# mikemey/cellcomm

Hardware: NVIDIA B200
Metric: BiGAN train cells/sec (higher is better)
Workload: dtype bf16

## Files before the change

### cellcomm_b200/_lib.py

```python
import ctypes as C
import os

from . import build as _build

_LIB = None

c_i32, c_i64, c_u32, c_u64, c_f32 = C.c_int32, C.c_int64, C.c_uint32, C.c_uint64, C.c_float
vp = C.c_void_p


class GemmDesc(C.Structure):
    _fields_ = [
        ("M", c_i32), ("N", c_i32),
        ("a_mn_major", c_i32), ("b_mn_major", c_i32),
        ("nseg", c_i32),
        ("a", vp * 4), ("lda", c_i64 * 4),
        ("b", vp * 4), ("ldb", c_i64 * 4),
        ("k", c_i32 * 4),
        ("alpha", c_f32),
        ("bias", vp), ("act", c_i32),
        ("dact_y", vp), ("ld_dact", c_i64), ("dact", c_i32),
        ("out16", vp), ("ld16", c_i64), ("beta16", c_i32),
        ("out32", vp), ("ld32", c_i64), ("beta32", c_i32),
        ("workspace", vp), ("workspace_elems", c_i64),
        ("force_splits", c_i32), ("force_bn", c_i32),
        ("rms_p32", vp), ("rms_ms", vp), ("rms_mom", vp), ("rms_p16", vp), ("rms_ld", c_i64),
        ("rms_lr", c_f32), ("rms_rho", c_f32), ("rms_momentum", c_f32), ("rms_eps", c_f32),
        ("route_world", c_i32), ("route_shard", c_i64), ("route_off0", c_i64),
        ("route_base", vp * 16),
        ("out16_lo", vp), ("ld16_lo", c_i64),
        ("rms_blocked", c_i32), ("rms_row0", c_i32), ("rms_p16_lo", vp),
    ]


class PeerRmspropDesc(C.Structure):
    _fields_ = [
        ("world", c_i32), ("rank", c_i32),
        ("grad", vp * 16), ("p16", vp * 16),
        ("p32", vp), ("ms", vp), ("mom", vp),
        ("start", c_i64), ("count", c_i64),
        ("broadcast", c_i32),
        ("lr", c_f32), ("rho", c_f32), ("momentum", c_f32), ("eps", c_f32),
        ("ready", vp), ("epoch", c_u32),
        ("epoch_ctr", vp),
        ("p16_multicast", vp),
        ("p16lo", vp * 16), ("p16lo_multicast", vp),
        ("lo_begin", c_i64 * 2), ("lo_end", c_i64 * 2),
    ]


ENC_MAX_OPS = ENC_MAX_SLOTS = 32
ENC_DENSE, ENC_SPLIT, ENC_COPY, ENC_BN_INFER, ENC_SOFTMAX = range(5)


class EncOp(C.Structure):
    _fields_ = [
        ("kind", c_i32), ("n_in", c_i32),
        ("in_", c_i32 * 4), ("w_row", c_i32 * 4),
        ("out", c_i32), ("out2", c_i32),
        ("width", c_i32), ("act", c_i32),
        ("w16", vp), ("ldw", c_i64),
        ("bias", vp),
        ("gamma", vp), ("beta", vp), ("mean", vp), ("var", vp),
        ("eps", c_f32),
# ... 13 lines not shown


SIGNATURES = {
    "cc_last_error": (C.c_char_p, []),
    "cc_version": (C.c_int, []),
    "cc_launch_count": (C.c_longlong, []),
    "cc_arch": (C.c_char_p, []),
    "cc_reload_env": (None, []),
    "cc_mtx_load_csr": (C.c_int, [C.c_char_p, C.POINTER(vp)]),
    "cc_coo_to_csr": (C.c_int, [vp, vp, vp, c_i64, C.POINTER(vp)]),
    "cc_csr_destroy": (None, [vp]),
    "cc_csr_rows": (c_i64, [vp]),
    "cc_csr_cols": (c_i64, [vp]),
    "cc_csr_nnz": (c_i64, [vp]),
    "cc_csr_rowptr": (vp, [vp]),
    "cc_csr_colidx": (vp, [vp]),
    "cc_csr_values": (vp, [vp]),
    "cc_csr_values64": (vp, [vp]),
    "cc_csr_row_ids": (vp, [vp]),
    "cc_csr_col_ids": (vp, [vp]),
    "cc_mtx_load_coo": (C.c_int, [C.c_char_p, C.POINTER(vp)]),
    "cc_coo_destroy": (None, [vp]),
    "cc_coo_nnz": (c_i64, [vp]),
    "cc_coo_gene": (vp, [vp]),
    "cc_coo_barcode": (vp, [vp]),
    "cc_coo_value": (vp, [vp]),
    "cc_coo_build_csr": (C.c_int, [vp, C.POINTER(vp)]),
    "cc_mtx_write": (C.c_int, [C.c_char_p, c_i64, c_i64, c_i64, vp, vp, vp, vp, vp]),
    "cc_encode_scratch_bytes": (c_i64, [C.POINTER(EncodePlan)]),
    "cc_encode_stream": (C.c_int, [vp, vp, vp, c_i64, c_i64, C.POINTER(EncodePlan), vp, c_i64, vp]),
    "cc_gather_rows": (C.c_int, [vp, vp, vp, vp, c_i64, c_i64, c_i64, vp, c_i64, vp, c_i64, vp]),
    "cc_gemm": (C.c_int, [C.POINTER(GemmDesc), vp]),
    "cc_gemm_workspace_elems": (c_i64, [c_i32, c_i32]),
    "cc_dense_fwd": (C.c_int, [c_i32, c_i32, c_i32, C.POINTER(vp), C.POINTER(c_i64),
                               C.POINTER(c_i32), C.POINTER(vp), C.POINTER(c_i64), vp, c_i32,
                               vp, c_i64, vp, c_i64, vp, c_i64, vp]),
    "cc_dense_dgrad": (C.c_int, [c_i32, c_i32, c_i32, C.POINTER(vp), C.POINTER(c_i64),
                                 C.POINTER(c_i32), C.POINTER(vp), C.POINTER(c_i64), vp, c_i64,
                                 c_i32, c_f32, vp, c_i64, c_i32, vp, c_i64, vp]),
    "cc_dense_wgrad": (C.c_int, [c_i32, c_i32, c_i32, vp, c_i64, vp, c_i64, vp, c_i64, c_i32, vp]),
    "cc_reduce_ws_floats": (c_i64, [c_i64, c_i64]),
    "cc_colsum": (C.c_int, [vp, c_i64, c_i64, c_i64, vp, c_i32, c_i32, vp]),
    "cc_colsum_ws": (C.c_int, [vp, c_i64, c_i64, c_i64, vp, c_i32, c_i32, vp, c_i64, vp]),
    "cc_bias_grad": (C.c_int, [vp, c_i64, vp, c_i64, c_i64, c_i64, c_i32, vp, c_i32, vp, c_i64, vp,
                               c_i64, c_i32, vp]),
    "cc_bias_grad_ws": (C.c_int, [vp, c_i64, vp, c_i64, c_i64, c_i64, c_i32, vp, c_i32, vp, c_i64,
                                  vp, c_i64, c_i32, vp, c_i64, vp]),
    "cc_split_bf16": (C.c_int, [vp, c_i64, vp, c_i64, vp, c_i64, c_i64, c_i64, c_i32, vp]),
    "cc_dropout": (C.c_int, [vp, c_i64, vp, c_i64, c_i64, c_i64, c_f32, vp, c_i64, c_u64, vp,
                             c_u32, c_i32, vp]),
    "cc_dropout_mask": (C.c_int, [vp, c_i64, c_i64, c_i64, c_f32, c_u64, vp, c_u32, vp]),
    "cc_uniform": (C.c_int, [vp, vp, c_i64, c_i64, c_i64, c_u64, vp, c_u32, vp]),
    "cc_counter_add": (C.c_int, [vp, c_u64, vp]),
    "cc_act_bwd": (C.c_int, [vp, c_i64, vp, c_i64, vp, c_i64, c_i64, c_i64, c_i32, c_i32, vp]),
    "cc_copy2d": (C.c_int, [vp, c_i64, vp, c_i64, c_i64, c_i64, c_i32, c_f32, c_i32, vp]),
    "cc_bn_stats": (C.c_int, [vp, c_i64, c_i64, c_i64, vp, c_i32, vp]),
    "cc_bn_stats_ws": (C.c_int, [vp, c_i64, c_i64, c_i64, vp, c_i32, vp, c_i64, vp]),
    "cc_bn_train_apply": (C.c_int, [vp, c_i64, vp, c_i64, c_i64, c_i64, vp, c_i64, vp, vp, c_f32,
                                    c_f32, vp, vp, vp, vp, c_i32, vp]),
    "cc_bn_infer": (C.c_int, [vp, c_i64, vp, c_i64, c_i64, c_i64, vp, vp, vp, vp, c_f32, c_i32,
                              vp]),
    "cc_bn_bwd_stats": (C.c_int, [vp, c_i64, vp, c_i64, c_i64, c_i64, vp, vp, vp, c_i32, vp]),
    "cc_bn_bwd_stats_ws": (C.c_int, [vp, c_i64, vp, c_i64, c_i64, c_i64, vp, vp, vp, c_i32, vp,
                                     c_i64, vp]),
    "cc_bn_bwd_apply": (C.c_int, [vp, c_i64, vp, c_i64, vp, c_i64, c_i64, c_i64, vp, vp, vp, vp,
                                  c_i64, vp, vp, c_i32, vp]),
# ... 62 lines not shown
```

### cellcomm_b200/csrc/gemm_sm100.cu

```cuda
#include <cuda.h>

#include <mutex>
#include <unordered_map>

#include "common.cuh"

namespace cc {

constexpr int BM = 128;
constexpr int BK = 64;
constexpr int UMMA_K = 16;
constexpr int MAX_SEG = CC_GEMM_MAX_SEG;

struct EpiParams {
  int M, N;
  float alpha;
  const float* bias;
  int act;
  const bf16* dact_y;
  long long ld_dact;
  int dact;
  bf16* out16;
  long long ld16;
  int beta16;
  bf16* out16_lo;
  long long ld16_lo;
  float* out32;
  long long ld32;
  int beta32;
  float* rms_p32;
  float* rms_ms;
  float* rms_mom;
  bf16* rms_p16;
  long long rms_ld;
  float rms_lr, rms_rho, rms_momentum, rms_eps;
  int rms_cs;
  int rms_blocked;
  int rms_row0;
  bf16* rms_p16lo;
  int rms_keep_operands;
  int route_world;
  unsigned int route_shard;
  long long route_off0;
  float* route_base[CC_PEER_MAX];
};

struct GemmParams {
  EpiParams epi;
  int nseg;
  int kblocks[MAX_SEG];
  int total_kblocks;
  int kb_per_split;
  int psplits;
  float* partial;
  long long partial_ld;
  long long partial_stride;
  unsigned long long adesc_hi, bdesc_hi;
  unsigned int a_kstep, b_kstep;
  unsigned int idesc;
  int bn_eff;
  int b_boxes;
  int b_half_rows;
  int cluster;
  int pair;
  unsigned int stage_tx;
};

struct TmaMaps {
  CUtensorMap a[MAX_SEG];
  CUtensorMap b[MAX_SEG];
};

__device__ __forceinline__ uint32_t smem_u32(const void* p) {
  return (uint32_t)__cvta_generic_to_shared(p);
}
__device__ __forceinline__ void mbar_init(uint32_t bar, uint32_t count) {
  asm volatile("mbarrier.init.shared::cta.b64 [%0], %1;" ::"r"(bar), "r"(count));
}
// ... 977 lines not shown
}

}
#include "wgrad_rmsprop_kernel.cuh"
namespace cc {

__global__ void splitk_finalize_kernel(const EpiParams e, const float* __restrict__ partial,
                                       long long partial_ld, long long partial_stride, int splits) {
  const int groups = (e.N + 3) / 4;
  const long long idx = (long long)blockIdx.x * blockDim.x + threadIdx.x;
  if (idx >= (long long)e.M * groups) return;
  const int r = (int)(idx / groups);
  const int c0 = (int)(idx % groups) * 4;
  const float* src = partial + (long long)r * partial_ld + c0;
  float4 a = make_float4(0.f, 0.f, 0.f, 0.f);
  for (int s0 = 0; s0 < splits; s0 += 8) {
    float4 q[8];
#pragma unroll
    for (int u = 0; u < 8; ++u)
      q[u] = (s0 + u < splits)
                 ? __ldcs(reinterpret_cast<const float4*>(src + (long long)(s0 + u) * partial_stride))
                 : make_float4(0.f, 0.f, 0.f, 0.f);
#pragma unroll
    for (int u = 0; u < 8; ++u) {
      if (s0 + u < splits) {
        a.x += q[u].x;
        a.y += q[u].y;
        a.z += q[u].z;
        a.w += q[u].w;
      }
    }
  }
  float v[4] = {a.x, a.y, a.z, a.w};
  const int ncols = min(4, e.N - c0);
#pragma unroll
  for (int j = 0; j < 4; ++j) {
    float x = v[j] * e.alpha;
    if (e.bias != nullptr && j < ncols) x += __ldg(e.bias + c0 + j);
    if (e.act == CC_ACT_SIGMOID) x = sigmoidf_(x);
    else if (e.act == CC_ACT_RELU) x = fmaxf(x, 0.f);
    v[j] = x;
  }
  if (e.dact != 0) {
    const bf16* yrow = e.dact_y + (long long)r * e.ld_dact + c0;
#pragma unroll
    for (int j = 0; j < 4; ++j) {
      if (j < ncols) {
        const float y = bf2f(yrow[j]);
        v[j] *= (e.dact == CC_ACT_SIGMOID) ? y * (1.f - y) : (y > 0.f ? 1.f : 0.f);
      }
    }
  }
  if (e.out32 != nullptr) {
    float* o = e.out32 + (long long)r * e.ld32 + c0;
    if (ncols == 4 && (((uintptr_t)o) & 15) == 0 && !e.beta32) {
      *reinterpret_cast<float4*>(o) = make_float4(v[0], v[1], v[2], v[3]);
    } else {
#pragma unroll
      for (int j = 0; j < 4; ++j)
        if (j < ncols) o[j] = e.beta32 ? o[j] + v[j] : v[j];
    }
  }
  if (e.out16 != nullptr) {
    bf16* o = e.out16 + (long long)r * e.ld16 + c0;
    if (ncols == 4 && (((uintptr_t)o) & 7) == 0 && !e.beta16) {
      __nv_bfloat162 p0 = __floats2bfloat162_rn(v[0], v[1]);
      __nv_bfloat162 p1 = __floats2bfloat162_rn(v[2], v[3]);
      uint2 u;
      u.x = *reinterpret_cast<uint32_t*>(&p0);
      u.y = *reinterpret_cast<uint32_t*>(&p1);
      *reinterpret_cast<uint2*>(o) = u;
    } else {
#pragma unroll
      for (int j = 0; j < 4; ++j)
        if (j < ncols) o[j] = f2bf(e.beta16 ? bf2f(o[j]) + v[j] : v[j]);
    }
    if (e.out16_lo != nullptr) {
      bf16* l = e.out16_lo + (long long)r * e.ld16_lo + c0;
#pragma unroll
      for (int j = 0; j < 4; ++j)
        if (j < ncols) l[j] = f2bf(v[j] - bf2f(f2bf(v[j])));
    }
  }
}

typedef CUresult (*PFN_encodeTiled)(CUtensorMap*, CUtensorMapDataType, cuuint32_t, void*,
                                    const cuuint64_t*, const cuuint64_t*, const cuuint32_t*,
                                    const cuuint32_t*, CUtensorMapInterleave, CUtensorMapSwizzle,
                                    CUtensorMapL2promotion, CUtensorMapFloatOOBfill);

static PFN_encodeTiled get_encode_fn() {
  static PFN_encodeTiled fn = nullptr;
  static std::once_flag once;
  std::call_once(once, [] {
    void* ptr = nullptr;
    cudaDriverEntryPointQueryResult qres;
    if (cudaGetDriverEntryPoint("cuTensorMapEncodeTiled", &ptr, cudaEnableDefault, &qres) ==
            cudaSuccess &&
        qres == cudaDriverEntryPointSuccess)
      fn = (PFN_encodeTiled)ptr;
  });
  return fn;
}

struct MapKey {
  const void* ptr;
  uint64_t inner, outer, ld;
  uint32_t box_inner, box_outer;
  uint32_t kind;
  bool operator==(const MapKey& o) const {
    return ptr == o.ptr && inner == o.inner && outer == o.outer && ld == o.ld &&
           box_inner == o.box_inner && box_outer == o.box_outer && kind == o.kind;
  }
};
struct MapKeyHash {
  size_t operator()(const MapKey& k) const {
// ... 330 lines not shown
  if (d->rms_blocked) {
    CC_REQUIRE(d->rms_p32 != nullptr && d->a_mn_major && d->b_mn_major && d->N > 128 &&
                   d->alpha == 1.f && d->bias == nullptr && d->act == 0 && d->dact_y == nullptr &&
                   d->out16 == nullptr && d->beta32 == 0 && d->route_world == 0 &&
                   d->force_splits <= 1 && (d->force_bn == 0 || d->force_bn == 256),
               "cc_gemm: rms_blocked is for plain weight-gradient GEMMs (X^T dZ, N > 128)");
    CC_REQUIRE(d->rms_row0 >= 0 && (d->rms_ld & 31) == 0 &&
                   ((((uintptr_t)d->rms_p32) | ((uintptr_t)d->rms_ms) | ((uintptr_t)d->rms_mom) |
                     ((uintptr_t)d->rms_p16) | ((uintptr_t)d->rms_p16_lo) | ((uintptr_t)d->out32)) & 15) == 0 &&
                   (d->out32 == nullptr || (d->ld32 & 3) == 0),
               "cc_gemm: rms_blocked needs 16-byte aligned blocks, rms_ld %% 32 == 0 (rms_ld=%lld)",
               (long long)d->rms_ld);
  }
  CC_REQUIRE(d->rms_p16_lo == nullptr || d->rms_blocked,
             "cc_gemm: rms_p16_lo is written by the blocked fused-optimiser epilogue only");
  if (d->route_world > 0) {
    CC_REQUIRE(d->out32 != nullptr && d->beta32 == 0 && d->workspace == nullptr &&
                   d->rms_p32 == nullptr,
               "cc_gemm: a routed output needs a plain fp32 output without split-K");
    CC_REQUIRE(d->route_shard > 0 && (d->route_shard & 7) == 0 && d->route_shard < (1ll << 32) &&
                   d->route_off0 >= 0 && (d->route_off0 & 3) == 0,
               "cc_gemm: route_shard=%lld route_off0=%lld", (long long)d->route_shard,
               (long long)d->route_off0);
    for (int q = 0; q < d->route_world; ++q)
      CC_REQUIRE(d->route_base[q] != nullptr, "cc_gemm: route_base[%d] is null", q);
  }
  if (g_num_sms == 0) {
    int dev = 0;
    CC_CHECK_CUDA(cudaGetDevice(&dev));
    CC_CHECK_CUDA(cudaDeviceGetAttribute(&g_num_sms, cudaDevAttrMultiProcessorCount, dev));
    const int cap = ENV.sms;
    if (cap >= 2 && cap < g_num_sms) g_num_sms = cap / 2 * 2;
  }
  const bool a_mn = d->a_mn_major != 0, b_mn = d->b_mn_major != 0;

  int bn = d->force_bn ? d->force_bn : ENV.bn;
  if (bn == 0) bn = (d->N > 128) ? 256 : 128;
  CC_REQUIRE(bn == 128 || bn == 256, "cc_gemm: BN=%d unsupported", bn);

  GemmParams p{};
  TmaMaps maps;
  memset(&maps, 0, sizeof(maps));
  p.nseg = d->nseg;
  int total = 0;
  for (int s = 0; s < d->nseg; ++s) {
    CC_REQUIRE(d->k[s] > 0, "cc_gemm: segment %d has k=%d", s, d->k[s]);
    p.kblocks[s] = (d->k[s] + BK - 1) / BK;
    total += p.kblocks[s];
  }
  p.total_kblocks = total;

  const int mt = (d->M + BM - 1) / BM;
  int nt = (d->N + bn - 1) / bn;
  int splits = 1;
  const long long Mpad = (long long)mt * BM, Npad = (long long)nt * bn;
  if (d->workspace != nullptr && d->rms_p32 == nullptr) {
    int want = d->force_splits ? d->force_splits : ENV.splits;
    if (want == 0) {
      const int tiles = mt * nt;
      if (2 * tiles <= g_num_sms && total >= 8) {
        want = (2 * g_num_sms) / tiles;
        if (want < 1) want = 1;
        if (want > total / 4) want = total / 4;
      } else {
        want = 1;
      }
// ... 50 lines not shown
  if (p.pair) {
    p.b_boxes = bn_eff / 128;
    p.stage_tx = (unsigned)(BM * BK * 2 + (bn_eff / 2) * BK * 2);
  }

  for (int s = 0; s < d->nseg; ++s) {
    int rc;
    if (a_mn)
      rc = make_map(&maps.a[s], d->a[s], (uint64_t)d->M, (uint64_t)d->k[s], (uint64_t)d->lda[s], 64, BK);
    else
      rc = make_map(&maps.a[s], d->a[s], (uint64_t)d->k[s], (uint64_t)d->M, (uint64_t)d->lda[s], BK, BM);
    if (rc) return rc;
    if (b_mn)
      rc = make_map(&maps.b[s], d->b[s], (uint64_t)d->N, (uint64_t)d->k[s], (uint64_t)d->ldb[s], 64, BK);
    else
      rc = make_map(&maps.b[s], d->b[s], (uint64_t)d->k[s], (uint64_t)d->N, (uint64_t)d->ldb[s], BK,
                    (uint32_t)(persistent ? (p.cluster == 2 ? bn_eff / 2 : bn_eff) : bn));
    if (rc) return rc;
  }

  const uint32_t mn_lbo = (uint32_t)ENV.mn_lbo;
  const uint32_t mn_sbo = (uint32_t)ENV.mn_sbo;
  const uint32_t mn_kstep = (uint32_t)ENV.mn_kstep;
  const uint32_t k_lbo = (uint32_t)ENV.k_lbo;
  const uint32_t k_sbo = (uint32_t)ENV.k_sbo;
  p.adesc_hi = a_mn ? desc_hi(mn_lbo, mn_sbo) : desc_hi(k_lbo, k_sbo);
  p.bdesc_hi = b_mn ? desc_hi(mn_lbo, mn_sbo) : desc_hi(k_lbo, k_sbo);
  p.a_kstep = a_mn ? mn_kstep : UMMA_K * 2;
  p.b_kstep = b_mn ? mn_kstep : UMMA_K * 2;
  p.idesc = (1u << 4) | (1u << 7) | (1u << 10) | ((a_mn ? 1u : 0u) << 15) |
            ((b_mn ? 1u : 0u) << 16) | ((uint32_t)((persistent ? bn_eff : bn) >> 3) << 17) |
            ((uint32_t)(((persistent && p.pair) ? 2 * BM : BM) >> 4) << 24);

  EpiParams& e = p.epi;
  e.M = d->M;
  e.N = d->N;
  e.alpha = d->alpha;
  e.bias = d->bias;
  e.act = d->act;
  e.dact_y = (const bf16*)d->dact_y;
  e.ld_dact = d->ld_dact;
  e.dact = d->dact_y ? d->dact : 0;
  e.out16 = (bf16*)d->out16;
  e.ld16 = d->ld16;
  e.beta16 = d->beta16;
  e.out16_lo = (bf16*)d->out16_lo;
  e.ld16_lo = d->ld16_lo;
  e.out32 = d->out32;
  e.ld32 = d->ld32;
  e.beta32 = d->beta32;
  e.rms_p32 = d->rms_p32;
  e.rms_ms = d->rms_ms;
  e.rms_mom = d->rms_mom;
  e.rms_p16 = (bf16*)d->rms_p16;
  e.rms_ld = d->rms_ld;
  e.rms_lr = d->rms_lr;
  e.rms_rho = d->rms_rho;
  e.rms_momentum = d->rms_momentum;
  e.rms_eps = d->rms_eps;
  e.rms_cs = (ENV.rms_cs ? 1 : 0) | (ENV.rms_l2_256 ? 8 : 0);
  e.rms_blocked = d->rms_blocked;
  e.rms_row0 = d->rms_row0;
  e.rms_p16lo = d->rms_blocked ? (bf16*)d->rms_p16_lo : nullptr;
  e.rms_keep_operands = ENV.rms_keep;
  e.route_world = d->route_world;
  e.route_shard = (unsigned)d->route_shard;
  e.route_off0 = d->route_off0;
  for (int q = 0; q < CC_PEER_MAX; ++q)
    e.route_base[q] = q < d->route_world ? d->route_base[q] : nullptr;

  if (persistent) {
    if (bn == 256 && d->rms_p32 != nullptr && a_mn && b_mn && d->alpha == 1.f &&
        d->bias == nullptr && d->act == 0 && e.dact == 0 && ENV.rms_warps == 8) {
      int nfast = ENV.rms_nfast;
      if (nfast < 0) nfast = ((long long)total * BK * d->N * 2 <= (48ll << 20)) ? 1 : 0;
      if (d->rms_blocked) {
        if (p.cluster == 2)
          return nfast ? launch_persistent_one<256, 4, true, true, false, 8, true, 2, false, true>(
                             maps, p, mt, nt, g_num_sms, st)
                       : launch_persistent_one<256, 4, true, true, false, 8, false, 2, false, true>(
                             maps, p, mt, nt, g_num_sms, st);
        return nfast ? launch_persistent_one<256, 4, true, true, false, 8, true, 1, false, true>(
                           maps, p, mt, nt, g_num_sms, st)
// ... 106 lines not shown
```

### cellcomm_b200/ops.py

```python
import ctypes as C

import torch

from . import _lib
from ._lib import GemmDesc, check

COMPUTE_DTYPE = torch.bfloat16
ACT_NONE, ACT_SIGMOID, ACT_RELU = 0, 1, 2
ACT_IDS = {None: 0, "none": 0, "linear": 0, "sigmoid": 1, "relu": 2}


def _stream():
    return torch.cuda.current_stream().cuda_stream


def _req(t, dtype, name):
    if t is None:
        return
    if not t.is_cuda:
        raise RuntimeError(f"cellcomm_b200.ops: {name} must be a CUDA tensor (no CPU fallback)")
    if t.dtype != dtype:
        raise TypeError(f"cellcomm_b200.ops: {name} must be {dtype}, got {t.dtype}")
    if t.dim() == 2 and t.shape[1] > 1 and t.stride(1) != 1:
        raise ValueError(f"cellcomm_b200.ops: {name} must be row-major (stride(1)==1)")
# ... 7 lines not shown
    if t is None:
        return 0
    if t.dim() == 1:
        return t.shape[0]
    return t.stride(0) if t.shape[0] > 1 else max(t.stride(0), t.shape[1])


def pad_ld(cols, mult=64):
    return max(mult, (cols + mult - 1) // mult * mult)


def alloc2d(rows, cols, dtype=torch.bfloat16, device="cuda", zero=True):
    ld = pad_ld(cols)
    buf = (torch.zeros if zero else torch.empty)((max(rows, 1), ld), dtype=dtype, device=device)
    return buf[:rows, :cols]


_WS = {}


def workspace(device):
    key = str(device)
    ws = _WS.get(key)
    if ws is None:
        ws = torch.empty(296 * 128 * 256 * 2, dtype=torch.float32, device=device)
        _WS[key] = ws
    return ws


def launch_count():
    return int(_lib.load().cc_launch_count())


def reload_env():
    _lib.load().cc_reload_env()


def gemm(M, N, a_list, b_list, k_list, a_mn, b_mn, *, bias=None, act=0, dact_y=None, dact=0,
         alpha=1.0, out16=None, beta16=0, out32=None, beta32=0, splits=0, bn=0, use_ws=True,
         rms=None, route=None, out16_lo=None, rms_row0=None, rms_lo=None):
    lib = _lib.load()
    d = GemmDesc()
    d.M, d.N = int(M), int(N)
    d.a_mn_major, d.b_mn_major = int(a_mn), int(b_mn)
    d.nseg = len(a_list)
    for s, (a, b, k) in enumerate(zip(a_list, b_list, k_list)):
        _req(a, torch.bfloat16, "A")
        _req(b, torch.bfloat16, "B")
        d.a[s], d.lda[s] = a.data_ptr(), _ld(a)
        d.b[s], d.ldb[s] = b.data_ptr(), _ld(b)
        d.k[s] = int(k)
    d.alpha = float(alpha)
    _req(bias, torch.float32, "bias")
    d.bias = _p(bias)
    d.act = int(act)
    _req(dact_y, torch.bfloat16, "dact_y")
    d.dact_y, d.ld_dact, d.dact = _p(dact_y), _ld(dact_y), int(dact)
    _req(out16, torch.bfloat16, "out16")
    _req(out32, torch.float32, "out32")
    d.out16, d.ld16, d.beta16 = _p(out16), _ld(out16), int(beta16)
    d.out32, d.ld32, d.beta32 = _p(out32), _ld(out32), int(beta32)
    if out16_lo is not None:
        _req(out16_lo, torch.bfloat16, "out16_lo")
        if out16 is None or beta16:
            raise ValueError("gemm(out16_lo=...): needs a plain bf16 out16 (the high-order term)")
        d.out16_lo, d.ld16_lo = out16_lo.data_ptr(), _ld(out16_lo)
    if use_ws:
        ws = workspace(a_list[0].device)
        d.workspace, d.workspace_elems = ws.data_ptr(), ws.numel()
    d.force_splits, d.force_bn = int(splits), int(bn)
    if rms is not None and rms_row0 is not None:
        p32, p16, ms, mom, lr, rho, momentum, eps = rms
        _req(p16, torch.bfloat16, "p16")
        if p16 is None or tuple(p16.shape) != (M, N):
            raise ValueError("gemm(rms=..., rms_row0=...): needs the [M, N] bf16 copy")
        ld = _ld(p16)
        need = (int(rms_row0) + M + 31) // 32 * 32 * ld
        for t, name in ((p32, "p32"), (ms, "ms"), (mom, "mom")):
            _req(t, torch.float32, name)
            if t.dim() != 1 or t.numel() < need:
                raise ValueError(f"gemm(rms_row0=...): {name} must be the layer's flat blocked array "
                                 f"of at least {need} elements")
        d.rms_p32, d.rms_ms, d.rms_mom, d.rms_p16 = p32.data_ptr(), ms.data_ptr(), \
            mom.data_ptr(), p16.data_ptr()
        d.rms_ld, d.rms_blocked, d.rms_row0 = ld, 1, int(rms_row0)
        if rms_lo is not None:
            _req(rms_lo, torch.bfloat16, "rms_lo")
            if tuple(rms_lo.shape) != (M, N) or _ld(rms_lo) != ld:
                raise ValueError("gemm(rms_lo=...): must be laid out like the bf16 copy")
            d.rms_p16_lo = rms_lo.data_ptr()
        d.rms_lr, d.rms_rho, d.rms_momentum, d.rms_eps = float(lr), float(rho), float(momentum), \
            float(eps)
    elif rms is not None:
        if rms_lo is not None:
            raise ValueError("gemm(rms_lo=...): only with the blocked state layout (rms_row0)")
        p32, p16, ms, mom, lr, rho, momentum, eps = rms
        for t, name in ((p32, "p32"), (ms, "ms"), (mom, "mom")):
            _req(t, torch.float32, name)
            if tuple(t.shape) != (M, N) or _ld(t) != _ld(p32):
                raise ValueError("gemm(rms=...): parameter / slot views must be [M, N] with one ld")
        d.rms_p32, d.rms_ms, d.rms_mom, d.rms_p16 = p32.data_ptr(), ms.data_ptr(), \
            mom.data_ptr(), _p(p16)
        if p16 is not None and _ld(p16) != _ld(p32):
# ... 377 lines not shown
```

### include/cellcomm_b200.h

```cpp
#ifndef CELLCOMM_B200_H
#define CELLCOMM_B200_H

#include <stddef.h>
#include <stdint.h>

#ifdef __cplusplus
extern "C" {
#endif

typedef void* cc_stream_t;

const char* cc_last_error(void);
int cc_version(void);
long long cc_launch_count(void);
const char* cc_arch(void);
void cc_reload_env(void);

typedef struct cc_csr cc_csr;

int cc_mtx_load_csr(const char* path, cc_csr** out);
int cc_coo_to_csr(const int64_t* gene, const int64_t* barcode, const double* val,
                  int64_t nnz, cc_csr** out);
void cc_csr_destroy(cc_csr* csr);
int64_t cc_csr_rows(const cc_csr* csr);
// ... 36 lines not shown
  int64_t ldb[CC_GEMM_MAX_SEG];
  int32_t k[CC_GEMM_MAX_SEG];
  float alpha;
  const float* bias;
  int32_t act;
  const void* dact_y;
  int64_t ld_dact;
  int32_t dact;
  void* out16;
  int64_t ld16;
  int32_t beta16;
  float* out32;
  int64_t ld32;
  int32_t beta32;
  float* workspace;
  int64_t workspace_elems;
  int32_t force_splits;
  int32_t force_bn;
  float* rms_p32;
  float* rms_ms;
  float* rms_mom;
  void* rms_p16;
  int64_t rms_ld;
  float rms_lr, rms_rho, rms_momentum, rms_eps;
  int32_t route_world;
  int64_t route_shard;
  int64_t route_off0;
  float* route_base[16];
  void* out16_lo;
  int64_t ld16_lo;
  int32_t rms_blocked;
  int32_t rms_row0;
  void* rms_p16_lo;
} cc_gemm_desc;

int cc_gemm(const cc_gemm_desc* desc, cc_stream_t stream);
int64_t cc_gemm_workspace_elems(int32_t M, int32_t N);

int cc_dense_fwd(int32_t M, int32_t N, int32_t nseg, const void* const* x, const int64_t* ldx,
                 const int32_t* k, const void* const* w, const int64_t* ldw, const float* bias,
                 int32_t act, void* out16, int64_t ld16, float* out32, int64_t ld32,
                 float* workspace, int64_t workspace_elems, cc_stream_t stream);
int cc_dense_dgrad(int32_t M, int32_t K, int32_t nseg, const void* const* dz, const int64_t* lddz,
                   const int32_t* n, const void* const* w, const int64_t* ldw, const void* dact_y,
                   int64_t ld_dact, int32_t dact, float alpha, void* out16, int64_t ld16,
                   int32_t beta16, float* workspace, int64_t workspace_elems, cc_stream_t stream);
int cc_dense_wgrad(int32_t M, int32_t K, int32_t N, const void* x, int64_t ldx, const void* dz,
                   int64_t lddz, float* dw, int64_t lddw, int32_t beta, cc_stream_t stream);


int64_t cc_reduce_ws_floats(int64_t rows, int64_t cols);

int cc_colsum(const void* x, int64_t ld, int64_t rows, int64_t cols, float* out, int32_t beta,
              int32_t dtypes, cc_stream_t stream);
int cc_colsum_ws(const void* x, int64_t ld, int64_t rows, int64_t cols, float* out, int32_t beta,
                 int32_t dtypes, float* ws, int64_t ws_floats, cc_stream_t stream);

int cc_bias_grad(const void* dy, int64_t lddy, const void* y, int64_t ldy, int64_t rows,
                 int64_t cols, int32_t act, float* out, int32_t beta, void* dz, int64_t lddz,
                 void* dz_lo, int64_t lddz_lo, int32_t dtypes, cc_stream_t stream);
int cc_bias_grad_ws(const void* dy, int64_t lddy, const void* y, int64_t ldy, int64_t rows,
                    int64_t cols, int32_t act, float* out, int32_t beta, void* dz, int64_t lddz,
                    void* dz_lo, int64_t lddz_lo, int32_t dtypes, float* ws, int64_t ws_floats,
                    cc_stream_t stream);
int cc_split_bf16(const void* x, int64_t ldx, void* hi, int64_t ldhi, void* lo, int64_t ldlo,
                  int64_t rows, int64_t cols, int32_t dtypes, cc_stream_t stream);

int cc_dropout(const void* x, int64_t ldx, void* out, int64_t ldo, int64_t rows, int64_t cols,
               float rate, const uint8_t* mask_u8, int64_t ldm, uint64_t seed,
               const uint64_t* counter_dev, uint32_t stream_id, int32_t dtypes,
// ... 153 lines not shown
```

Measured before the change: 59020.

## Add mma.sync small-GEMM kernel with split-K tickets for small shapes

Adds a separate 64x64x64 cp.async + ldmatrix + mma.sync GEMM kernel. cc_gemm routes small problems to it by default: narrow-N, short-K row-major products, and small-tile, long-K weight-gradient products, which use split-K with a last-arriver ticket reduction. The epilogue code moves into a shared header so both kernels use it. The aim is to avoid the tcgen05/TMA persistent kernel's setup and tile underuse on tiny GEMMs. The cost is a second code path, with ticket counters in global memory that must reset correctly.

New measurement: 59230, median of 6. About the same (+0.4%).

```diff
diff --git a/cellcomm_b200/_lib.py b/cellcomm_b200/_lib.py
--- a/cellcomm_b200/_lib.py
+++ b/cellcomm_b200/_lib.py
@@ -30,6 +30,7 @@
         ("route_base", vp * 16),
         ("out16_lo", vp), ("ld16_lo", c_i64),
         ("rms_blocked", c_i32), ("rms_row0", c_i32), ("rms_p16_lo", vp),
+        ("force_path", c_i32),
     ]
 
 
@@ -109,6 +110,7 @@
     "cc_gather_rows": (C.c_int, [vp, vp, vp, vp, c_i64, c_i64, c_i64, vp, c_i64, vp, c_i64, vp]),
     "cc_gemm": (C.c_int, [C.POINTER(GemmDesc), vp]),
     "cc_gemm_workspace_elems": (c_i64, [c_i32, c_i32]),
+    "cc_gemm_small_tickets_pending": (c_i64, []),
     "cc_dense_fwd": (C.c_int, [c_i32, c_i32, c_i32, C.POINTER(vp), C.POINTER(c_i64),
                                C.POINTER(c_i32), C.POINTER(vp), C.POINTER(c_i64), vp, c_i32,
                                vp, c_i64, vp, c_i64, vp, c_i64, vp]),
diff --git a/cellcomm_b200/csrc/gemm_epilogue.cuh b/cellcomm_b200/csrc/gemm_epilogue.cuh
--- /dev/null
+++ b/cellcomm_b200/csrc/gemm_epilogue.cuh
@@ -0,0 +1,116 @@
+#pragma once
+#include "common.cuh"
+
+namespace cc {
+
+struct EpiParams {
+  int M, N;
+  float alpha;
+  const float* bias;
+  int act;
+  const bf16* dact_y;
+  long long ld_dact;
+  int dact;
+  bf16* out16;
+  long long ld16;
+  int beta16;
+  bf16* out16_lo;
+  long long ld16_lo;
+  float* out32;
+  long long ld32;
+  int beta32;
+  float* rms_p32;
+  float* rms_ms;
+  float* rms_mom;
+  bf16* rms_p16;
+  long long rms_ld;
+  float rms_lr, rms_rho, rms_momentum, rms_eps;
+  int rms_cs;
+  int rms_blocked;
+  int rms_row0;
+  bf16* rms_p16lo;
+  int rms_keep_operands;
+  int route_world;
+  unsigned int route_shard;
+  long long route_off0;
+  float* route_base[CC_PEER_MAX];
+};
+
+inline EpiParams epi_from_desc(const cc_gemm_desc* d) {
+  EpiParams e{};
+  e.M = d->M;
+  e.N = d->N;
+  e.alpha = d->alpha;
+  e.bias = d->bias;
+  e.act = d->act;
+  e.dact_y = (const bf16*)d->dact_y;
+  e.ld_dact = d->ld_dact;
+  e.dact = d->dact_y ? d->dact : 0;
+  e.out16 = (bf16*)d->out16;
+  e.ld16 = d->ld16;
+  e.beta16 = d->beta16;
+  e.out16_lo = (bf16*)d->out16_lo;
+  e.ld16_lo = d->ld16_lo;
+  e.out32 = d->out32;
+  e.ld32 = d->ld32;
+  e.beta32 = d->beta32;
+  return e;
+}
+
+__device__ __forceinline__ void epilogue_store4(const EpiParams& e, int r, int c0, float (&v)[4]) {
+  const int ncols = min(4, e.N - c0);
+#pragma unroll
+  for (int j = 0; j < 4; ++j) {
+    float x = v[j] * e.alpha;
+    if (e.bias != nullptr && j < ncols) x += __ldg(e.bias + c0 + j);
+    if (e.act == CC_ACT_SIGMOID) x = sigmoidf_(x);
+    else if (e.act == CC_ACT_RELU) x = fmaxf(x, 0.f);
+    v[j] = x;
+  }
+  if (e.dact != 0) {
+    const bf16* yrow = e.dact_y + (long long)r * e.ld_dact + c0;
+#pragma unroll
+    for (int j = 0; j < 4; ++j) {
+      if (j < ncols) {
+        const float y = bf2f(yrow[j]);
+        v[j] *= (e.dact == CC_ACT_SIGMOID) ? y * (1.f - y) : (y > 0.f ? 1.f : 0.f);
+      }
+    }
+  }
+  if (e.out32 != nullptr) {
+    float* o = e.out32 + (long long)r * e.ld32 + c0;
+    if (ncols == 4 && (((uintptr_t)o) & 15) == 0 && !e.beta32) {
+      *reinterpret_cast<float4*>(o) = make_float4(v[0], v[1], v[2], v[3]);
+    } else {
+#pragma unroll
+      for (int j = 0; j < 4; ++j)
+        if (j < ncols) o[j] = e.beta32 ? o[j] + v[j] : v[j];
+    }
+  }
+  if (e.out16 != nullptr) {
+    bf16* o = e.out16 + (long long)r * e.ld16 + c0;
+    if (ncols == 4 && (((uintptr_t)o) & 7) == 0 && !e.beta16) {
+      __nv_bfloat162 p0 = __floats2bfloat162_rn(v[0], v[1]);
+      __nv_bfloat162 p1 = __floats2bfloat162_rn(v[2], v[3]);
+      uint2 u;
+      u.x = *reinterpret_cast<uint32_t*>(&p0);
+      u.y = *reinterpret_cast<uint32_t*>(&p1);
+      *reinterpret_cast<uint2*>(o) = u;
+    } else {
+#pragma unroll
+      for (int j = 0; j < 4; ++j)
+        if (j < ncols) o[j] = f2bf(e.beta16 ? bf2f(o[j]) + v[j] : v[j]);
+    }
+    if (e.out16_lo != nullptr) {
+      bf16* l = e.out16_lo + (long long)r * e.ld16_lo + c0;
+#pragma unroll
+      for (int j = 0; j < 4; ++j)
+        if (j < ncols) l[j] = f2bf(v[j] - bf2f(f2bf(v[j])));
+    }
+  }
+}
+
+int gemm_small(const cc_gemm_desc* d, int num_sms, cudaStream_t st);
+bool gemm_small_wanted(const cc_gemm_desc* d);
+
+}
diff --git a/cellcomm_b200/csrc/gemm_sm100.cu b/cellcomm_b200/csrc/gemm_sm100.cu
--- a/cellcomm_b200/csrc/gemm_sm100.cu
+++ b/cellcomm_b200/csrc/gemm_sm100.cu
@@ -4,6 +4,7 @@
 #include <unordered_map>
 
 #include "common.cuh"
+#include "gemm_epilogue.cuh"
 
 namespace cc {
 
@@ -11,39 +12,6 @@
 constexpr int BK = 64;
 constexpr int UMMA_K = 16;
 constexpr int MAX_SEG = CC_GEMM_MAX_SEG;
-
-struct EpiParams {
-  int M, N;
-  float alpha;
-  const float* bias;
-  int act;
-  const bf16* dact_y;
-  long long ld_dact;
-  int dact;
-  bf16* out16;
-  long long ld16;
-  int beta16;
-  bf16* out16_lo;
-  long long ld16_lo;
-  float* out32;
-  long long ld32;
-  int beta32;
-  float* rms_p32;
-  float* rms_ms;
-  float* rms_mom;
-  bf16* rms_p16;
-  long long rms_ld;
-  float rms_lr, rms_rho, rms_momentum, rms_eps;
-  int rms_cs;
-  int rms_blocked;
-  int rms_row0;
-  bf16* rms_p16lo;
-  int rms_keep_operands;
-  int route_world;
-  unsigned int route_shard;
-  long long route_off0;
-  float* route_base[CC_PEER_MAX];
-};
 
 struct GemmParams {
   EpiParams epi;
@@ -1087,56 +1055,7 @@
     }
   }
   float v[4] = {a.x, a.y, a.z, a.w};
-  const int ncols = min(4, e.N - c0);
-#pragma unroll
-  for (int j = 0; j < 4; ++j) {
-    float x = v[j] * e.alpha;
-    if (e.bias != nullptr && j < ncols) x += __ldg(e.bias + c0 + j);
-    if (e.act == CC_ACT_SIGMOID) x = sigmoidf_(x);
-    else if (e.act == CC_ACT_RELU) x = fmaxf(x, 0.f);
-    v[j] = x;
-  }
-  if (e.dact != 0) {
-    const bf16* yrow = e.dact_y + (long long)r * e.ld_dact + c0;
-#pragma unroll
-    for (int j = 0; j < 4; ++j) {
-      if (j < ncols) {
-        const float y = bf2f(yrow[j]);
-        v[j] *= (e.dact == CC_ACT_SIGMOID) ? y * (1.f - y) : (y > 0.f ? 1.f : 0.f);
-      }
-    }
-  }
-  if (e.out32 != nullptr) {
-    float* o = e.out32 + (long long)r * e.ld32 + c0;
-    if (ncols == 4 && (((uintptr_t)o) & 15) == 0 && !e.beta32) {
-      *reinterpret_cast<float4*>(o) = make_float4(v[0], v[1], v[2], v[3]);
-    } else {
-#pragma unroll
-      for (int j = 0; j < 4; ++j)
-        if (j < ncols) o[j] = e.beta32 ? o[j] + v[j] : v[j];
-    }
-  }
-  if (e.out16 != nullptr) {
-    bf16* o = e.out16 + (long long)r * e.ld16 + c0;
-    if (ncols == 4 && (((uintptr_t)o) & 7) == 0 && !e.beta16) {
-      __nv_bfloat162 p0 = __floats2bfloat162_rn(v[0], v[1]);
-      __nv_bfloat162 p1 = __floats2bfloat162_rn(v[2], v[3]);
-      uint2 u;
-      u.x = *reinterpret_cast<uint32_t*>(&p0);
-      u.y = *reinterpret_cast<uint32_t*>(&p1);
-      *reinterpret_cast<uint2*>(o) = u;
-    } else {
-#pragma unroll
-      for (int j = 0; j < 4; ++j)
-        if (j < ncols) o[j] = f2bf(e.beta16 ? bf2f(o[j]) + v[j] : v[j]);
-    }
-    if (e.out16_lo != nullptr) {
-      bf16* l = e.out16_lo + (long long)r * e.ld16_lo + c0;
-#pragma unroll
-      for (int j = 0; j < 4; ++j)
-        if (j < ncols) l[j] = f2bf(v[j] - bf2f(f2bf(v[j])));
-    }
-  }
+  epilogue_store4(e, r, c0, v);
 }
 
 typedef CUresult (*PFN_encodeTiled)(CUtensorMap*, CUtensorMapDataType, cuuint32_t, void*,
@@ -1533,6 +1452,12 @@
     const int cap = ENV.sms;
     if (cap >= 2 && cap < g_num_sms) g_num_sms = cap / 2 * 2;
   }
+  CC_REQUIRE(d->force_path >= 0 && d->force_path <= 2, "cc_gemm: force_path=%d", d->force_path);
+  if (d->force_path == 2) return gemm_small(d, g_num_sms, st);
+  if (d->force_path == 0 && d->rms_p32 == nullptr && d->route_world == 0 && d->force_bn == 0 &&
+      d->force_splits == 0 && ENV.bn == 0 && ENV.splits == 0 && ENV.bn_eff == 0 && ENV.pair == 0 &&
+      gemm_small_wanted(d))
+    return gemm_small(d, g_num_sms, st);
   const bool a_mn = d->a_mn_major != 0, b_mn = d->b_mn_major != 0;
 
   int bn = d->force_bn ? d->force_bn : ENV.bn;
@@ -1649,23 +1574,8 @@
             ((b_mn ? 1u : 0u) << 16) | ((uint32_t)((persistent ? bn_eff : bn) >> 3) << 17) |
             ((uint32_t)(((persistent && p.pair) ? 2 * BM : BM) >> 4) << 24);
 
+  p.epi = epi_from_desc(d);
   EpiParams& e = p.epi;
-  e.M = d->M;
-  e.N = d->N;
-  e.alpha = d->alpha;
-  e.bias = d->bias;
-  e.act = d->act;
-  e.dact_y = (const bf16*)d->dact_y;
-  e.ld_dact = d->ld_dact;
-  e.dact = d->dact_y ? d->dact : 0;
-  e.out16 = (bf16*)d->out16;
-  e.ld16 = d->ld16;
-  e.beta16 = d->beta16;
-  e.out16_lo = (bf16*)d->out16_lo;
-  e.ld16_lo = d->ld16_lo;
-  e.out32 = d->out32;
-  e.ld32 = d->ld32;
-  e.beta32 = d->beta32;
   e.rms_p32 = d->rms_p32;
   e.rms_ms = d->rms_ms;
   e.rms_mom = d->rms_mom;
diff --git a/cellcomm_b200/csrc/gemm_small.cu b/cellcomm_b200/csrc/gemm_small.cu
--- /dev/null
+++ b/cellcomm_b200/csrc/gemm_small.cu
@@ -0,0 +1,337 @@
+#include <algorithm>
+
+#include "gemm_epilogue.cuh"
+
+namespace cc {
+
+constexpr int SM_BM = 64, SM_BN = 64, SM_BK = 64;
+constexpr int SM_STAGES = 3;
+constexpr int SM_THREADS = 128;
+constexpr int SM_LD = 72;
+constexpr int SM_TILE = 64 * SM_LD;
+constexpr int SM_SMEM = SM_STAGES * 2 * SM_TILE * 2;
+constexpr int SM_OUT_LD = 72;
+static_assert(SM_BM * SM_OUT_LD * 4 <= SM_SMEM, "output tile aliases the operand ring");
+constexpr int SM_MAX_SPLITS = 16;
+constexpr int SM_TICKETS = 4096;
+
+__device__ unsigned int g_small_tickets[SM_TICKETS];
+
+struct SmallParams {
+  EpiParams epi;
+  int nseg;
+  const bf16* a[CC_GEMM_MAX_SEG];
+  long long lda[CC_GEMM_MAX_SEG];
+  const bf16* b[CC_GEMM_MAX_SEG];
+  long long ldb[CC_GEMM_MAX_SEG];
+  int k[CC_GEMM_MAX_SEG];
+  int kb_start[CC_GEMM_MAX_SEG + 1];
+  int kb_per_split;
+  float* partial;
+};
+
+__device__ __forceinline__ uint32_t smem_addr(const void* p) {
+  return (uint32_t)__cvta_generic_to_shared(p);
+}
+__device__ __forceinline__ void cp_async16(uint32_t dst, const void* src, int bytes) {
+  asm volatile("cp.async.cg.shared.global [%0], [%1], 16, %2;" ::"r"(dst), "l"(src), "r"(bytes)
+               : "memory");
+}
+__device__ __forceinline__ void cp_async_commit() {
+  asm volatile("cp.async.commit_group;" ::: "memory");
+}
+template <int N>
+__device__ __forceinline__ void cp_async_wait() {
+  asm volatile("cp.async.wait_group %0;" ::"n"(N) : "memory");
+}
+__device__ __forceinline__ void ldsm_x4(uint32_t addr, uint32_t (&r)[4]) {
+  asm volatile("ldmatrix.sync.aligned.m8n8.x4.shared.b16 {%0, %1, %2, %3}, [%4];"
+               : "=r"(r[0]), "=r"(r[1]), "=r"(r[2]), "=r"(r[3])
+               : "r"(addr));
+}
+__device__ __forceinline__ void ldsm_x4_t(uint32_t addr, uint32_t (&r)[4]) {
+  asm volatile("ldmatrix.sync.aligned.m8n8.x4.trans.shared.b16 {%0, %1, %2, %3}, [%4];"
+               : "=r"(r[0]), "=r"(r[1]), "=r"(r[2]), "=r"(r[3])
+               : "r"(addr));
+}
+__device__ __forceinline__ void mma_bf16(float (&c)[4], const uint32_t (&a)[4], uint32_t b0,
+                                         uint32_t b1) {
+  asm volatile(
+      "mma.sync.aligned.m16n8k16.row.col.f32.bf16.bf16.f32 {%0, %1, %2, %3}, {%4, %5, %6, %7}, "
+      "{%8, %9}, {%0, %1, %2, %3};"
+      : "+f"(c[0]), "+f"(c[1]), "+f"(c[2]), "+f"(c[3])
+      : "r"(a[0]), "r"(a[1]), "r"(a[2]), "r"(a[3]), "r"(b0), "r"(b1));
+}
+
+template <bool MN>
+__device__ __forceinline__ void load_tile(bf16* tile, const bf16* base, long long ld, int rows,
+                                          int r0, int kseg, int k0) {
+#pragma unroll
+  for (int j = 0; j < (64 * 8) / SM_THREADS; ++j) {
+    const int i = threadIdx.x + j * SM_THREADS;
+    const int t_row = i >> 3, t_col = (i & 7) * 8;
+    int row, col, lim_row, lim_col;
+    if (MN) {
+      row = k0 + t_row;  lim_row = kseg;
+      col = r0 + t_col;  lim_col = rows;
+    } else {
+      row = r0 + t_row;  lim_row = rows;
+      col = k0 + t_col;  lim_col = kseg;
+    }
+    int n = row < lim_row ? min(8, lim_col - col) : 0;
+    if (n < 0) n = 0;
+    const bf16* src = n > 0 ? base + (long long)row * ld + col : base;
+    cp_async16(smem_addr(tile + t_row * SM_LD + t_col), src, 2 * n);
+  }
+}
+
+template <bool A_MN, bool B_MN>
+__global__ void __launch_bounds__(SM_THREADS, 4)
+gemm_small_kernel(const __grid_constant__ SmallParams p) {
+  extern __shared__ __align__(128) uint8_t sm_raw[];
+  bf16* sm = reinterpret_cast<bf16*>(sm_raw);
+  auto a_tile = [&](int s) { return sm + (2 * s) * SM_TILE; };
+  auto b_tile = [&](int s) { return sm + (2 * s + 1) * SM_TILE; };
+
+  const int warp = threadIdx.x >> 5, lane = threadIdx.x & 31;
+  const int wm = (warp >> 1) * 32, wn = (warp & 1) * 32;
+  const int m0 = blockIdx.x * SM_BM, n0 = blockIdx.y * SM_BN;
+  const int total_kb = p.kb_start[p.nseg];
+  const int kb_begin = blockIdx.z * p.kb_per_split;
+  const int kb_end = min(total_kb, kb_begin + p.kb_per_split);
+  const int nkb = kb_end - kb_begin;
+
+  auto load_stage = [&](int kb, int s) {
+    int seg = 0;
+    while (seg < p.nseg - 1 && kb >= p.kb_start[seg + 1]) ++seg;
+    const int k0 = (kb - p.kb_start[seg]) * SM_BK;
+    load_tile<A_MN>(a_tile(s), p.a[seg], p.lda[seg], p.epi.M, m0, p.k[seg], k0);
+    load_tile<B_MN>(b_tile(s), p.b[seg], p.ldb[seg], p.epi.N, n0, p.k[seg], k0);
+  };
+
+  float acc[2][4][4];
+#pragma unroll
+  for (int i = 0; i < 2; ++i)
+#pragma unroll
+    for (int j = 0; j < 4; ++j)
+#pragma unroll
+      for (int q = 0; q < 4; ++q) acc[i][j][q] = 0.f;
+
+#pragma unroll
+  for (int s = 0; s < SM_STAGES - 1; ++s) {
+    if (s < nkb) load_stage(kb_begin + s, s);
+    cp_async_commit();
+  }
+  const int lq = lane >> 3, lr = lane & 7;
+  for (int i = 0; i < nkb; ++i) {
+    cp_async_wait<SM_STAGES - 2>();
+    __syncthreads();
+    if (i + SM_STAGES - 1 < nkb) load_stage(kb_begin + i + SM_STAGES - 1, (i + SM_STAGES - 1) % SM_STAGES);
+    cp_async_commit();
+    const bf16* at = a_tile(i % SM_STAGES);
+    const bf16* bt = b_tile(i % SM_STAGES);
+#pragma unroll
+    for (int kk = 0; kk < SM_BK; kk += 16) {
+      uint32_t af[2][4], bfr[2][4];
+#pragma unroll
+      for (int mt = 0; mt < 2; ++mt) {
+        const int mrow = wm + mt * 16 + (lq & 1) * 8, kcol = kk + (lq >> 1) * 8;
+        if (A_MN) ldsm_x4_t(smem_addr(at + (kcol + lr) * SM_LD + mrow), af[mt]);
+        else      ldsm_x4(smem_addr(at + (mrow + lr) * SM_LD + kcol), af[mt]);
+      }
+#pragma unroll
+      for (int np = 0; np < 2; ++np) {
+        const int ncol = wn + np * 16 + (lq >> 1) * 8, kcol = kk + (lq & 1) * 8;
+        if (B_MN) ldsm_x4_t(smem_addr(bt + (kcol + lr) * SM_LD + ncol), bfr[np]);
+        else      ldsm_x4(smem_addr(bt + (ncol + lr) * SM_LD + kcol), bfr[np]);
+      }
+#pragma unroll
+      for (int mt = 0; mt < 2; ++mt)
+#pragma unroll
+        for (int nt = 0; nt < 4; ++nt)
+          mma_bf16(acc[mt][nt], af[mt], bfr[nt >> 1][(nt & 1) * 2], bfr[nt >> 1][(nt & 1) * 2 + 1]);
+    }
+  }
+  cp_async_wait<0>();
+  __syncthreads();
+
+  float* out = reinterpret_cast<float*>(sm_raw);
+  {
+    const int g = lane >> 2, t = lane & 3;
+#pragma unroll
+    for (int mt = 0; mt < 2; ++mt)
+#pragma unroll
+      for (int nt = 0; nt < 4; ++nt) {
+        const int r = wm + mt * 16 + g, c = wn + nt * 8 + 2 * t;
+        *reinterpret_cast<float2*>(out + r * SM_OUT_LD + c) = make_float2(acc[mt][nt][0], acc[mt][nt][1]);
+        *reinterpret_cast<float2*>(out + (r + 8) * SM_OUT_LD + c) =
+            make_float2(acc[mt][nt][2], acc[mt][nt][3]);
+      }
+  }
+  __syncthreads();
+  constexpr int GROUPS = SM_BM * SM_BN / 4 / SM_THREADS;
+  if (gridDim.z == 1) {
+#pragma unroll
+    for (int j = 0; j < GROUPS; ++j) {
+      const int i = threadIdx.x + j * SM_THREADS;
+      const int r = i >> 4, c = (i & 15) * 4;
+      if (m0 + r < p.epi.M && n0 + c < p.epi.N) {
+        const float4 q = *reinterpret_cast<const float4*>(out + r * SM_OUT_LD + c);
+        float v[4] = {q.x, q.y, q.z, q.w};
+        epilogue_store4(p.epi, m0 + r, n0 + c, v);
+      }
+    }
+    return;
+  }
+
+  const int tile = blockIdx.y * gridDim.x + blockIdx.x;
+  const int splits = gridDim.z;
+  float* tile_part = p.partial + (long long)tile * splits * (SM_BM * SM_BN);
+  {
+    float* mine = tile_part + (long long)blockIdx.z * (SM_BM * SM_BN);
+#pragma unroll
+    for (int j = 0; j < GROUPS; ++j) {
+      const int i = threadIdx.x + j * SM_THREADS;
+      const int r = i >> 4, c = (i & 15) * 4;
+      __stcg(reinterpret_cast<float4*>(mine + r * SM_BN + c),
+             *reinterpret_cast<const float4*>(out + r * SM_OUT_LD + c));
+    }
+  }
+  __threadfence();
+  __syncthreads();
+  __shared__ bool last;
+  if (threadIdx.x == 0) last = atomicAdd(&g_small_tickets[tile], 1u) == (unsigned)splits - 1u;
+  __syncthreads();
+  if (!last) return;
+  __threadfence();
+#pragma unroll
+  for (int h = 0; h < GROUPS; h += GROUPS / 2) {
+    float4 sum[GROUPS / 2];
+#pragma unroll
+    for (int j = 0; j < GROUPS / 2; ++j) sum[j] = make_float4(0.f, 0.f, 0.f, 0.f);
+    for (int s0 = 0; s0 < splits; s0 += 4) {
+      float4 q[4][GROUPS / 2];
+#pragma unroll
+      for (int u = 0; u < 4; ++u)
+#pragma unroll
+        for (int j = 0; j < GROUPS / 2; ++j) {
+          const int i = threadIdx.x + (h + j) * SM_THREADS;
+          q[u][j] = s0 + u < splits
+                        ? __ldcg(reinterpret_cast<const float4*>(
+                              tile_part + (long long)(s0 + u) * (SM_BM * SM_BN) + (i >> 4) * SM_BN +
+                              (i & 15) * 4))
+                        : make_float4(0.f, 0.f, 0.f, 0.f);
+        }
+#pragma unroll
+      for (int u = 0; u < 4; ++u) {
+        if (s0 + u < splits) {
+#pragma unroll
+          for (int j = 0; j < GROUPS / 2; ++j) {
+            sum[j].x += q[u][j].x;
+            sum[j].y += q[u][j].y;
+            sum[j].z += q[u][j].z;
+            sum[j].w += q[u][j].w;
+          }
+        }
+      }
+    }
+#pragma unroll
+    for (int j = 0; j < GROUPS / 2; ++j) {
+      const int i = threadIdx.x + (h + j) * SM_THREADS;
+      const int r = i >> 4, c = (i & 15) * 4;
+      if (m0 + r < p.epi.M && n0 + c < p.epi.N) {
+        float v[4] = {sum[j].x, sum[j].y, sum[j].z, sum[j].w};
+        epilogue_store4(p.epi, m0 + r, n0 + c, v);
+      }
+    }
+  }
+  if (threadIdx.x == 0) g_small_tickets[tile] = 0u;
+}
+
+template <bool A_MN, bool B_MN>
+static int launch_small(const SmallParams& p, dim3 grid, cudaStream_t st) {
+  auto kern = gemm_small_kernel<A_MN, B_MN>;
+  static bool attr_set = false;
+  if (!attr_set) {
+    CC_CHECK_CUDA(cudaFuncSetAttribute(kern, cudaFuncAttributeMaxDynamicSharedMemorySize, SM_SMEM));
+    attr_set = true;
+  }
+  kern<<<grid, SM_THREADS, SM_SMEM, st>>>(p);
+  CC_CHECK_LAUNCH();
+  return 0;
+}
+
+constexpr int SMALL_MIN_N = 8;
+constexpr int SMALL_MAX_N = 256;
+constexpr int SMALL_MAX_ROW_KBLOCKS = 6;
+constexpr int SMALL_MAX_WGRAD_TILES = 25;
+constexpr long long SMALL_MAX_WGRAD_FLOP = 1ll << 31;
+constexpr int SMALL_MIN_WGRAD_K = 4096;
+
+bool gemm_small_wanted(const cc_gemm_desc* d) {
+  long long ksum = 0, kblocks = 0;
+  for (int s = 0; s < d->nseg; ++s) {
+    ksum += d->k[s];
+    kblocks += (d->k[s] + SM_BK - 1) / SM_BK;
+  }
+  if (!d->a_mn_major)
+    return d->b_mn_major && d->N >= SMALL_MIN_N && d->N <= SMALL_MAX_N &&
+           kblocks <= SMALL_MAX_ROW_KBLOCKS;
+  const long long tiles = (long long)((d->M + SM_BM - 1) / SM_BM) * ((d->N + SM_BN - 1) / SM_BN);
+  return tiles <= SMALL_MAX_WGRAD_TILES && ksum >= SMALL_MIN_WGRAD_K &&
+         2ll * d->M * d->N * ksum <= SMALL_MAX_WGRAD_FLOP;
+}
+
+int gemm_small(const cc_gemm_desc* d, int num_sms, cudaStream_t st) {
+  CC_REQUIRE(d->rms_p32 == nullptr && d->route_world == 0,
+             "cc_gemm: the small-GEMM kernel has no fused optimiser or routed output");
+  SmallParams p{};
+  p.epi = epi_from_desc(d);
+  p.nseg = d->nseg;
+  int total = 0;
+  for (int s = 0; s < d->nseg; ++s) {
+    CC_REQUIRE(d->k[s] > 0, "cc_gemm: segment %d has k=%d", s, d->k[s]);
+    CC_REQUIRE((((uintptr_t)d->a[s] | (uintptr_t)d->b[s]) & 15) == 0 && d->lda[s] % 8 == 0 &&
+                   d->ldb[s] % 8 == 0,
+               "cc_gemm: segment %d operands need 16-byte aligned bases and rows (lda=%lld ldb=%lld)",
+               s, (long long)d->lda[s], (long long)d->ldb[s]);
+    p.a[s] = (const bf16*)d->a[s];
+    p.lda[s] = d->lda[s];
+    p.b[s] = (const bf16*)d->b[s];
+    p.ldb[s] = d->ldb[s];
+    p.k[s] = d->k[s];
+    p.kb_start[s] = total;
+    total += (d->k[s] + SM_BK - 1) / SM_BK;
+  }
+  p.kb_start[d->nseg] = total;
+  const int mt = (d->M + SM_BM - 1) / SM_BM, nt = (d->N + SM_BN - 1) / SM_BN;
+  const long long tiles = (long long)mt * nt;
+  int splits = 1;
+  if (d->a_mn_major && d->workspace != nullptr && tiles <= SM_TICKETS) {
+    long long want = (4ll * num_sms) / tiles;
+    want = std::min<long long>(want, std::min(total / 4, SM_MAX_SPLITS));
+    want = std::min<long long>(want, d->workspace_elems / (tiles * SM_BM * SM_BN));
+    if (want >= 2) splits = (int)want;
+  }
+  p.kb_per_split = (total + splits - 1) / splits;
+  splits = (total + p.kb_per_split - 1) / p.kb_per_split;
+  p.partial = splits > 1 ? d->workspace : nullptr;
+  CC_REQUIRE(nt <= 65535, "cc_gemm: N=%d is too wide for the small-GEMM kernel", d->N);
+  const dim3 grid((unsigned)mt, (unsigned)nt, (unsigned)splits);
+  const bool a_mn = d->a_mn_major != 0, b_mn = d->b_mn_major != 0;
+  if (a_mn) return b_mn ? launch_small<true, true>(p, grid, st) : launch_small<true, false>(p, grid, st);
+  return b_mn ? launch_small<false, true>(p, grid, st) : launch_small<false, false>(p, grid, st);
+}
+
+}
+
+extern "C" int64_t cc_gemm_small_tickets_pending(void) {
+  unsigned int h[cc::SM_TICKETS];
+  if (cudaMemcpyFromSymbol(h, cc::g_small_tickets, sizeof(h)) != cudaSuccess) {
+    cc::set_error("cc_gemm_small_tickets_pending: cannot read the ticket counters");
+    return -1;
+  }
+  int64_t n = 0;
+  for (unsigned int v : h) n += v;
+  return n;
+}
diff --git a/cellcomm_b200/ops.py b/cellcomm_b200/ops.py
--- a/cellcomm_b200/ops.py
+++ b/cellcomm_b200/ops.py
@@ -63,13 +63,20 @@
     return int(_lib.load().cc_launch_count())
 
 
+def gemm_small_tickets_pending():
+    n = int(_lib.load().cc_gemm_small_tickets_pending())
+    if n < 0:
+        check(-1)
+    return n
+
+
 def reload_env():
     _lib.load().cc_reload_env()
 
 
 def gemm(M, N, a_list, b_list, k_list, a_mn, b_mn, *, bias=None, act=0, dact_y=None, dact=0,
          alpha=1.0, out16=None, beta16=0, out32=None, beta32=0, splits=0, bn=0, use_ws=True,
-         rms=None, route=None, out16_lo=None, rms_row0=None, rms_lo=None):
+         rms=None, route=None, out16_lo=None, rms_row0=None, rms_lo=None, path=0):
     lib = _lib.load()
     d = GemmDesc()
     d.M, d.N = int(M), int(N)
@@ -99,7 +106,7 @@
     if use_ws:
         ws = workspace(a_list[0].device)
         d.workspace, d.workspace_elems = ws.data_ptr(), ws.numel()
-    d.force_splits, d.force_bn = int(splits), int(bn)
+    d.force_splits, d.force_bn, d.force_path = int(splits), int(bn), int(path)
     if rms is not None and rms_row0 is not None:
         p32, p16, ms, mom, lr, rho, momentum, eps = rms
         _req(p16, torch.bfloat16, "p16")
diff --git a/include/cellcomm_b200.h b/include/cellcomm_b200.h
--- a/include/cellcomm_b200.h
+++ b/include/cellcomm_b200.h
@@ -92,10 +92,12 @@
   int32_t rms_blocked;
   int32_t rms_row0;
   void* rms_p16_lo;
+  int32_t force_path;
 } cc_gemm_desc;
 
 int cc_gemm(const cc_gemm_desc* desc, cc_stream_t stream);
 int64_t cc_gemm_workspace_elems(int32_t M, int32_t N);
+int64_t cc_gemm_small_tickets_pending(void);
 
 int cc_dense_fwd(int32_t M, int32_t N, int32_t nseg, const void* const* x, const int64_t* ldx,
                  const int32_t* k, const void* const* w, const int64_t* ldw, const float* bias,
```
